# victorramirez952/tomography_3d_reconstructor

Hardware: NVIDIA B200
Metric: Gvoxels/s mask-stack->mesh+volume (higher is better)
Workload: dtype u8 -> bit-packed u32 (topology), f64 field taps -> f32 vertices

## Files before the change

include/t3d.h:

```cpp
#ifndef T3D_H
#define T3D_H

#include <stdint.h>

#ifdef __cplusplus
extern "C" {
#endif

const char* t3d_last_error(void);
int t3d_version(void);
int64_t t3d_words_per_row(int W);
int64_t t3d_launch_count(void);
void t3d_count_launches(int n);


int t3d_pack_masks(const void* masks_u8, int Z, int H, int W, int threshold, void* bits, void* stream);

int t3d_pack_gap(const void* masks_u8, int Z, int H, int W, int threshold, void* bits, void* counts_u64, void* bbox_u32x6,
                 void* stream);

int t3d_unpack_bits(const void* bits, int Z, int H, int W, void* out_u8, void* stream);

int64_t t3d_fill_holes_scratch_bytes(int n_planes, int H, int W);
int t3d_fill_holes_2d(void* bits, int n_planes, int64_t plane_stride_words, int H, int W, void* scratch, void* stream);
// ... 55 lines not shown
int64_t t3d_canonicalize_workspace_bytes(int64_t V, int64_t F);
int t3d_mesh_canonicalize(const void* verts_in, int64_t V, const void* faces_in, int64_t F, void* verts_out,
                          void* faces_out_i64, void* faces_out_i32, void* counts_u64, void* workspace, void* stream);

int64_t t3d_canonicalize_fast_workspace_bytes(int64_t V, int64_t F);
int t3d_mesh_canonicalize_fast_dev(const void* verts_in, int64_t V_cap, const void* V_dev_u64, const void* faces_in, int64_t F_cap,
                                   const void* F_dev_u64, void* verts_out, void* faces_out_i64, void* faces_out_i32,
                                   void* counts_u64, void* workspace, void* stream);
int64_t t3d_canonicalize_structured_workspace_bytes(int64_t V, int64_t F, uint32_t cap_z, uint32_t cap_g0, int Zs);
int t3d_mesh_canonicalize_structured_dev(const void* verts_in, const void* vkeys_u64, int64_t V_cap, const void* sizes_u64,
                                         const void* V_dev_u64, int Zs, int Hs, int Ws, const void* chunkbase_u32,
                                         const void* aw_base_u32, uint32_t aw_stride, int z_offset, int unpad_shift,
                                         const void* cum_f64, const void* adj_f64, int n_cum, int zkey_bits, uint32_t cap_z,
                                         uint32_t cap_g0, const void* faces_in, int64_t F_cap, const void* F_dev_u64,
                                         void* verts_out, void* faces_out_i64, void* faces_out_i32, void* counts_u64,
                                         void* n_g0_u64, void* workspace, int phases, void* stream);

int64_t t3d_mesh_measure_workspace_bytes(void);
int t3d_mesh_measure_dev(const void* verts_f32, const void* faces, int64_t F_cap, const void* F_dev_u64, int faces_are_i64,
                         void* out_f64, void* workspace, void* stream);

int64_t t3d_reconstruct_workspace_bytes(int Z, int H, int W, int add_padding, int n_stages, uint32_t cap_active,
                                        uint32_t cap_verts, uint32_t cap_faces, uint32_t cap_zverts, uint32_t cap_g0);
int64_t t3d_reconstruct_results_len(int Z);
int t3d_reconstruct(const void* masks_u8, int Z, int H, int W, int threshold, int close_ends, int n_stages, unsigned erode_mask,
                    int add_padding, const double* weights3_host, const void* cum_f64, const void* adj_f64, int n_cum,
                    double mm_per_pixel_y, double mm_per_pixel_x, int scale_in_f64, uint32_t cap_active, uint32_t cap_verts,
                    uint32_t cap_faces, uint32_t cap_zverts, uint32_t cap_g0, int zkey_bits, void* verts_out_f32,
                    void* faces_out_i64, void* results_u64, void* workspace, void* stream);

int t3d_slab_pack_gap_ok(const void* masks_u8, int n_own, int H, int W, int threshold);
// ... 70 lines not shown
```

tomography_3d_reconstructor_b200/_lib.py:

```python
from __future__ import annotations

import ctypes
import os

_HERE = os.path.dirname(os.path.abspath(__file__))
LIB_PATH = os.path.join(_HERE, "libt3d.so")

_c = ctypes
_vp, _i, _i64, _u32, _dbl = _c.c_void_p, _c.c_int, _c.c_int64, _c.c_uint32, _c.c_double

class McField(ctypes.Structure):
    _fields_ = [("occ_bits", _vp), ("Z", _i), ("H", _i), ("W", _i), ("pad", _i), ("gaussian", _i), ("weights3_host", _vp),
                ("field_f32", _vp), ("level", _dbl)]


SIGNATURES = {
    "t3d_last_error": (_c.c_char_p, []),
    "t3d_version": (_i, []),
    "t3d_words_per_row": (_i64, [_i]),
    "t3d_launch_count": (_i64, []),
    "t3d_count_launches": (None, [_i]),
    "t3d_pack_masks": (_i, [_vp, _i, _i, _i, _i, _vp, _vp]),
    "t3d_pack_gap": (_i, [_vp, _i, _i, _i, _i, _vp, _vp, _vp, _vp]),
    "t3d_unpack_bits": (_i, [_vp, _i, _i, _i, _vp, _vp]),
# ... 13 lines not shown
    "t3d_field_dense": (_i, [_vp, _i, _i, _i, _i, _i, _vp, _vp, _vp]),
    "t3d_cube_cases": (_i, [_vp, _i, _i, _i, _vp, _vp]),
    "t3d_canonicalize_workspace_bytes": (_i64, [_i64, _i64]),
    "t3d_mesh_canonicalize": (_i, [_vp, _i64, _vp, _i64, _vp, _vp, _vp, _vp, _vp, _vp]),
    "t3d_canonicalize_fast_workspace_bytes": (_i64, [_i64, _i64]),
    "t3d_mesh_measure_workspace_bytes": (_i64, []),
    "t3d_exclusive_scan_u32_dev": (_i, [_vp, _vp, _i64, _i64, _i, _i, _i, _vp, _vp, _vp, _vp]),
    "t3d_mc_words_dev": (_i, [_vp, _i, _i, _i, _i, _i, _vp, _vp, _u32, _vp, _vp, _vp, _vp, _vp, _vp]),
    "t3d_mc_emit_dev": (_i, [_vp, _i, _i, _i, _i, _i, _vp, _vp, _vp, _vp, _u32, _vp, _u32, _u32, _vp, _vp, _i, _vp, _vp]),
    "t3d_mc_vertices_dev": (_i, [_vp, _i, _i, _i, _i, _i, _vp, _vp, _dbl, _vp, _vp, _u32, _i, _i, _vp, _vp, _i, _dbl, _dbl, _i, _i, _vp,
                                 _vp]),
    "t3d_mesh_canonicalize_fast_dev": (_i, [_vp, _i64, _vp, _vp, _i64, _vp, _vp, _vp, _vp, _vp, _vp, _vp]),
    "t3d_mesh_measure_dev": (_i, [_vp, _vp, _i64, _vp, _i, _vp, _vp, _vp]),
    "t3d_canonicalize_structured_workspace_bytes": (_i64, [_i64, _i64, _u32, _u32, _i]),
    "t3d_mesh_canonicalize_structured_dev": (_i, [_vp, _vp, _i64, _vp, _vp, _i, _i, _i, _vp, _vp, _u32, _i, _i, _vp, _vp, _i, _i, _u32,
                                                  _u32, _vp, _i64, _vp, _vp, _vp, _vp, _vp, _vp, _vp, _i, _vp]),
    "t3d_reconstruct_workspace_bytes": (_i64, [_i, _i, _i, _i, _i, _u32, _u32, _u32, _u32, _u32]),
    "t3d_reconstruct_results_len": (_i64, [_i]),
    "t3d_reconstruct": (_i, [_vp, _i, _i, _i, _i, _i, _i, _c.c_uint, _i, _vp, _vp, _vp, _i, _dbl, _dbl, _i, _u32, _u32, _u32,
                             _u32, _u32, _i, _vp, _vp, _vp, _vp, _vp]),
    "t3d_reconstruct_slab_workspace_bytes": (_i64, [_i, _i, _i, _i, _i, _i, _i, _u32, _u32, _u32, _u32, _u32]),
    "t3d_slab_pack_gap_ok": (_i, [_vp, _i, _i, _i, _i]),
    "t3d_slab_pack": (_i, [_vp, _i, _i, _i, _i, _i, _i, _i, _i, _vp, _vp, _vp, _vp, _vp]),
    "t3d_reconstruct_slab": (_i, [_vp, _i, _i, _i, _i, _i, _i, _c.c_uint, _i, _i, _i, _i, _i, _c.c_float, _i, _c.c_float, _i, _vp, _vp,
                                  _vp, _i, _dbl, _dbl, _i, _u32, _u32, _u32, _u32, _u32, _i, _vp, _vp, _vp, _vp, _vp, _vp, _vp]),
    "t3d_slab_stitch_faces": (_i, [_vp, _i64, _vp, _i64, _i, _vp]),
    "t3d_edt_workspace_bytes": (_i64, [_i, _i, _i]),
    "t3d_edt_xy_workspace_bytes": (_i64, [_i, _i, _i]),
    "t3d_edt_xy": (_i, [_vp, _i, _i, _i, _i, _vp, _vp, _vp, _vp]),
    "t3d_edt_z_workspace_bytes": (_i64, [_i, _i, _i]),
    "t3d_edt_z": (_i, [_vp, _vp, _i, _i, _i, _vp, _c.c_float, _i, _vp, _vp, _vp]),
# ... 53 lines not shown
```

tomography_3d_reconstructor_b200/csrc/t3d_common.cuh:

```cuda
#pragma once
#include <cuda_runtime.h>
#include <stdint.h>
#include <stdio.h>

int t3d_num_sms(void);
#define T3D_NUM_SMS (t3d_num_sms())
bool t3d_first_use_on_device(int slot);
enum { T3D_ONCE_FILL_HOLES_ATTR = 0, T3D_ONCE_MC_LUTS = 1, T3D_ONCE_SORT_ATTR = 2, T3D_ONCE_MORPH4_ATTR = 3, T3D_ONCE_SLOTS = 8 };

extern "C" void t3d_set_error(const char* fmt, ...);
extern "C" void t3d_count_launches(int n);
int t3d_zero_async(void* p, size_t n, cudaStream_t st);
void t3d_prezero_register(const void* p, size_t n);
void t3d_prezero_clear(void);
void t3d_canonicalize_structured_zero_range(int64_t V, int64_t F, uint32_t cap_z, uint32_t cap_g0, int Zs, int64_t* offset,
                                            int64_t* size);

#define T3D_CHECK_LAUNCH(name)                                                                   \
    do {                                                                                         \
        cudaError_t e__ = cudaGetLastError();                                                    \
        if (e__ != cudaSuccess) {                                                                \
            t3d_set_error("%s: launch failed: %s", name, cudaGetErrorString(e__));               \
            return 1;                                                                            \
        }                                                                                        \
// ... 120 lines not shown
```

tomography_3d_reconstructor_b200/csrc/t3d_pipeline.cu:

```cuda
#include <stdint.h>

#include <stdlib.h>

#include <nvtx3/nvToolsExt.h>

#include "t3d.h"
#include "t3d_field.cuh"

struct NvtxRange {
    bool open;
    explicit NvtxRange(const char* name) : open(true) { nvtxRangePushA(name); }
    void end() { if (open) { nvtxRangePop(); open = false; } }
    ~NvtxRange() { end(); }
};

enum {
    R_NACTIVE = 0, R_NX = 1, R_NY = 2, R_NZ = 3, R_NT = 4, R_VCANON = 5, R_FCANON = 6, R_UNVERIFIED = 7, R_OVERFLOW = 8,
    R_NAMBIGUOUS = 9, R_NEXACT = 10, R_VOLUME_F64 = 11, R_AREA_F64 = 12, R_BBOX_I32X6 = 13 , R_VRAW = 16, R_NEXC = 17,
    R_NGHOST = 18, R_NLEAD = 19, R_NG0 = 25,
    R_COUNTS = 32
};

#define EXC_CAP (1u << 20)
#define SURF_HALO 3
// ... 335 lines not shown
    r_mc.end();
    marks.mark("vertices", st);
    NvtxRange r_canon("t3d:ensure_manifold_mesh+measures");
    T3D_CUDA(cudaEventRecord(side->e[4], st));
    T3D_CUDA(cudaStreamWaitEvent(side->s, side->e[4], 0));
    RUN(t3d_mc_emit_view_dev(view, x_off, ws + L.sign, Zp, Hp, Wp, g.z_begin, g.z_end, ws + L.ballots, ws + L.chunkbase, ws + L.aw_idx,
                             ws + L.aw_base, cap_active, R + R_NACTIVE, cap_verts, cap_faces, ws + L.vkeys, ws + L.faces_raw, 2, side->s));
    T3D_CUDA(cudaEventRecord(side->e[6], side->s));
    RUN(t3d_mesh_measure_dev(ws + L.verts_raw, ws + L.faces_raw, cap_faces, R + R_NT, 0, R + R_VOLUME_F64, ws + L.measure, side->s));
    T3D_CUDA(cudaEventRecord(side->e[5], side->s));
    t3d_canon_faces_ready_event(side->e[6]);
    if (cap_zverts)
        RUN(t3d_mesh_canonicalize_structured_dev(ws + L.verts_raw, ws + L.vkeys, cap_verts, R + R_NACTIVE, R + R_VRAW, Zp, Hp, Wp,
                                                 ws + L.chunkbase, ws + L.aw_base, cap_active, g.z_offset, 1, cum_f64, adj_f64, n_cum,
                                                 zkey_bits, cap_zverts, cap_g0, ws + L.faces_raw, cap_faces, R + R_NT, verts_out_f32,
                                                 faces_out_i64, nullptr, R + R_VCANON, R + R_NG0, ws + L.canon, 3, st));
    else
        RUN(t3d_mesh_canonicalize_fast_dev(ws + L.verts_raw, cap_verts, R + R_VRAW, ws + L.faces_raw, cap_faces, R + R_NT,
                                           verts_out_f32, faces_out_i64, nullptr, R + R_VCANON, ws + L.canon, st));
    if (t3d_canon_faces_ready_pending()) T3D_CUDA(cudaStreamWaitEvent(st, side->e[6], 0));
    if (g.want_ghost || g.want_lead)
        k_count_plane_vertices<<<1, 64, 0, st>>>((const float*)verts_out_f32, R + R_VCANON, g.z_ghost, g.z_lead, g.want_ghost,
                                                 g.want_lead, R + R_NGHOST, R + R_NLEAD);
    if (g.want_ghost || g.want_lead) t3d_count_launches(1);
    marks.mark("canonicalize", st);
    T3D_CUDA(cudaStreamWaitEvent(st, side->e[5], 0));
    marks.mark("wait measures", st);
    marks.report(st);
    return 0;
}

// ... 275 lines not shown
```

tomography_3d_reconstructor_b200/csrc/t3d_surface.cu:

```cuda
#include <stdlib.h>

#include <cub/device/device_radix_sort.cuh>

#include "t3d_field.cuh"

#define FY 8

__device__ __noinline__ uint32_t exact_sign_bits(const OccView* v, int zp, int yp, int wp, uint32_t need, uint32_t s)
{
    while (need) {
        const int b = __ffs(need) - 1;
        need &= need - 1;
        if (field_value(*v, zp, yp, (wp << 5) + b) > 0.5f) s |= 1u << b; else s &= ~(1u << b);
    }
    return s;
}

__device__ __forceinline__ uint4 prow4(const OccView& v, int zp, int yp, int wp4, uint32_t& left, uint32_t& right)
{
    const int z = zp - v.pad, y = yp - v.pad;
    if (z < 0 || z >= v.Z || y < 0 || y >= v.H) { left = right = 0u; return make_uint4(0, 0, 0, 0); }
    const uint32_t* row = v.bits + (z * v.ps + (long long)y * v.rs);
    const int w0 = 4 * wp4;
    const uint4 o = (w0 < v.nw) ? *reinterpret_cast<const uint4*>(row + w0) : make_uint4(0, 0, 0, 0);
// ... 751 lines not shown

struct CanonS {
    const float* verts;
    const unsigned long long* vkeys;
    const unsigned long long* sizes;
    uint32_t cap_verts, cap_z, cap_g0;
    int Zs, Hs;
    int ncr;
    const uint32_t* chunkbase;
    const uint32_t* aw_base;
    uint32_t stride;
    int g_plane;
    int z_offset; float shift;
    const double* cum; const double* adj; int n_cum;
    int zkey_bits;
    unsigned long long* zkeys;
    uint32_t* zval;
    const uint32_t* zperm;
    unsigned long long* gkeys;
    uint32_t* gval;
    const uint32_t* gperm;
    uint32_t* perm;
    unsigned long long* n_g0_out;
};

template <int AX>
__device__ __forceinline__ uint32_t before_row(const CanonS& c, int64_t row)
{
    const uint32_t na = (uint32_t)c.sizes[0];
    const uint32_t r = row >= (int64_t)c.Zs * c.Hs ? na : c.chunkbase[row * c.ncr];
    return r >= na ? (uint32_t)c.sizes[1 + AX] : c.aw_base[(int64_t)AX * c.stride + r];
}

// ... 30 lines not shown
__device__ __forceinline__ uint32_t canon_zkey(const CanonS& c, uint32_t i, uint32_t nx, uint32_t ny, uint32_t gZ)
{
    if (i < gZ) return 0u;
    const uint32_t raw = nx + ny + i;
    const int k = (int)(c.vkeys[raw] >> 42);
    uint32_t zk = float_key(c.verts[3 * (int64_t)raw]);
    if (c.zkey_bits < 32) {
        const uint32_t base = float_key(plane_z(c, k));
        zk = zk >= base ? zk - base : 0u;
        const uint32_t lim = (1u << c.zkey_bits) - 1u;
        zk = zk > lim ? lim : zk;
    }
    return zk;
}

template <int ZS_U, typename KeyT, typename KeyFn, typename ValFn>
__device__ __forceinline__ void cta_radix_sort_u(uint32_t n, int passes, KeyFn key_of, ValFn value_of, KeyT* keyA, KeyT* keyB, uint32_t* idxA,
                                               uint32_t* idxB, uint32_t* out)
{
    __shared__ uint32_t s_hist[ZS_WARPS][256];
    __shared__ uint32_t s_tot[256];
    __shared__ uint32_t s_carry[8];
    const int tid = threadIdx.x, w = tid >> 5, lane = tid & 31;
    const uint32_t per = (((n + ZS_WARPS - 1) / ZS_WARPS) + 31u) & ~31u;
    const uint32_t ws = min(n, (uint32_t)w * per), we = min(n, ws + per);
    const KeyT* kin = keyA; const uint32_t* iin = idxA;
    KeyT* kout = keyB; uint32_t* iout = idxB;
    for (int p = 0; p < passes; ++p) {
        const int shift = 8 * p;
        const bool first = p == 0, last = p == passes - 1;
        for (int i = tid; i < ZS_WARPS * 256; i += ZS_THREADS) (&s_hist[0][0])[i] = 0;
        __syncthreads();
        for (uint32_t i0 = ws + lane; i0 < we; i0 += 32 * ZS_U) {
            KeyT kk[ZS_U];
#pragma unroll
            for (int u = 0; u < ZS_U; ++u) {
                const uint32_t i = i0 + 32 * u;
                if (i < we) { if (first) { kk[u] = key_of(i); keyA[i] = kk[u]; } else kk[u] = kin[i]; }
            }
#pragma unroll
            for (int u = 0; u < ZS_U; ++u)
                if (i0 + 32 * u < we) atomicAdd(&s_hist[w][(uint32_t)(kk[u] >> shift) & 255u], 1u);
        }
        __syncthreads();
        if (tid < 256) {
            uint32_t t = 0;
            for (int ww = 0; ww < ZS_WARPS; ++ww) t += s_hist[ww][tid];
            s_tot[tid] = t;
        }
        __syncthreads();
        if (tid < 256) {
            const uint32_t v = s_tot[tid];
            const uint32_t incl = warp_incl_scan(v);
            if (lane == 31) s_carry[w] = incl;
            asm volatile("bar.sync 1, 256;" ::: "memory");
            uint32_t carry = 0;
            for (int ww = 0; ww < w; ++ww) carry += s_carry[ww];
            uint32_t run = carry + incl - v;
            for (int ww = 0; ww < ZS_WARPS; ++ww) { const uint32_t h = s_hist[ww][tid]; s_hist[ww][tid] = run; run += h; }
        }
        __syncthreads();
        for (uint32_t c0 = ws; c0 < we; c0 += 32 * ZS_U) {
            KeyT kk[ZS_U];
            uint32_t ii[ZS_U];
#pragma unroll
            for (int u = 0; u < ZS_U; ++u) {
                const uint32_t i = c0 + 32 * u + lane;
                kk[u] = 0; ii[u] = 0;
                if (i < we) {
                    kk[u] = first ? keyA[i] : kin[i];
                    ii[u] = first ? value_of(i) : iin[i];
                }
            }
#pragma unroll
            for (int u = 0; u < ZS_U; ++u) {
                if (c0 + 32 * u >= we) break;
                const uint32_t i = c0 + 32 * u + lane;
                const bool ok = i < we;
                const KeyT key = kk[u];
                const uint32_t idx = ii[u];
                const uint32_t d = ok ? ((uint32_t)(key >> shift) & 255u) : 0xffffffffu;
                const uint32_t peers = __match_any_sync(0xffffffffu, d);
                const uint32_t rank = __popc(peers & ((1u << lane) - 1u));
                uint32_t pos = 0;
                if (ok) pos = s_hist[w][d] + rank;
                __syncwarp();
                if (ok && rank == 0) s_hist[w][d] += __popc(peers);
                __syncwarp();
                if (ok) {
                    if (last) out[pos] = idx;
                    else { kout[pos] = key; iout[pos] = idx; }
                }
            }
        }
        __syncthreads();
        const KeyT* tk = kin; const uint32_t* ti = iin;
        kin = kout; iin = iout;
        kout = (KeyT*)tk; iout = (uint32_t*)ti;
    }
}

template <int ZS_U>
__global__ void __launch_bounds__(ZS_THREADS) k_zsort_layers(CanonS c, uint32_t* __restrict__ keyA, uint32_t* __restrict__ keyB,
                                                            uint32_t* __restrict__ idxA, uint32_t* __restrict__ idxB,
                                                            uint32_t* __restrict__ zperm)
{
    const uint32_t nx = (uint32_t)c.sizes[1], ny = (uint32_t)c.sizes[2], nz = (uint32_t)c.sizes[3];
    if ((unsigned long long)nx + ny + nz > c.cap_verts || nz > c.cap_z) return;
    const int layer = blockIdx.x;
    uint32_t s = before_row<2>(c, (int64_t)layer * c.Hs), e = before_row<2>(c, (int64_t)(layer + 1) * c.Hs);
    if (e > nz) e = nz;
    if (s >= e) return;
    const uint32_t n = e - s;
    uint32_t gX, gY, gZ;
    g0_sizes(c, gX, gY, gZ);
    if (n == 1 || e <= gZ) {
        for (uint32_t i = s + threadIdx.x; i < e; i += ZS_THREADS) zperm[i] = i;
        return;
    }
    cta_radix_sort_u<ZS_U, uint32_t>(n, (c.zkey_bits + 7) / 8, [&](uint32_t i) { return canon_zkey(c, s + i, nx, ny, gZ); },
                                     [&](uint32_t i) { return s + i; }, keyA + s, keyB + s, idxA + s, idxB + s, zperm + s);
}

__global__ void __launch_bounds__(ZS_THREADS) k_gsort(CanonS c, unsigned long long* __restrict__ keyA, unsigned long long* __restrict__ keyB,
                                                     uint32_t* __restrict__ idxA, uint32_t* __restrict__ idxB, uint32_t* __restrict__ gperm)
{
    const uint32_t nx = (uint32_t)c.sizes[1], ny = (uint32_t)c.sizes[2], nz = (uint32_t)c.sizes[3];
    if ((unsigned long long)nx + ny + nz > c.cap_verts) return;
    uint32_t gX, gY, gZ;
    g0_sizes(c, gX, gY, gZ);
    const uint32_t n = gX + gY + gZ;
    if (n == 0 || n > c.cap_g0) return;
    auto raw_of = [&](uint32_t t) -> uint32_t { return t < gX ? t : t < gX + gY ? nx + (t - gX) : nx + ny + (t - gX - gY); };
    if (n == 1) { if (threadIdx.x == 0) gperm[0] = raw_of(0); return; }
    cta_radix_sort_u<1, unsigned long long>(n, 8, [&](uint32_t t) {
        const float* v = c.verts + 3 * (int64_t)raw_of(t);
        return ((unsigned long long)float_key(v[1]) << 32) | float_key(v[2]);
    }, raw_of, keyA, keyB, idxA, idxB, gperm);
}

__global__ void __launch_bounds__(256) k_canon_positions(CanonS c)
{
    __shared__ uint32_t s_g[3];
    const uint32_t i = blockIdx.x * blockDim.x + threadIdx.x;
    const uint32_t nx = (uint32_t)c.sizes[1], ny = (uint32_t)c.sizes[2], nz = (uint32_t)c.sizes[3];
    const unsigned long long V64 = (unsigned long long)nx + ny + nz;
    if (V64 > c.cap_verts) return;
    if (threadIdx.x == 0) g0_sizes(c, s_g[0], s_g[1], s_g[2]);
    __syncthreads();
    if (i >= (uint32_t)V64) return;
    if (nz > c.cap_z) { c.perm[i] = i; return; }
    const uint32_t gX = s_g[0], gY = s_g[1], gZ = s_g[2];
    const uint32_t nG = gX + gY + gZ;
    if (i == 0 && c.n_g0_out) *c.n_g0_out = nG;
    if (i < nG) c.perm[i] = (nG <= c.cap_g0) ? c.gperm[i] : (i < gX ? i : i < gX + gY ? nx + (i - gX) : nx + ny + (i - gX - gY));
    if (i < nx) {
        if (i < gX) return;
        const unsigned long long key = c.vkeys[i];
        const int k = (int)(key >> 42), j = (int)((key >> 22) & 0xfffffu);
        c.perm[i + before_row<1>(c, (int64_t)k * c.Hs + j) + before_row<2>(c, (int64_t)k * c.Hs)] = i;
    } else if (i < nx + ny) {
        const uint32_t iy = i - nx;
        if (iy < gY) return;
        const unsigned long long key = c.vkeys[i];
        const int k = (int)(key >> 42), j = (int)((key >> 22) & 0xfffffu);
        const int64_t row = (int64_t)k * c.Hs + j;
        const uint32_t lo = before_row<1>(c, row), hi = before_row<1>(c, row + 1);
        const uint32_t mine = float_key(c.verts[3 * (int64_t)i + 1]);
        uint32_t r = 0;
        for (uint32_t e = lo; e < hi; ++e) {
            const uint32_t ke = float_key(c.verts[3 * (int64_t)(nx + e) + 1]);
            r += (ke < mine || (ke == mine && e < iy)) ? 1u : 0u;
        }
        c.perm[before_row<0>(c, row + 1) + lo + r + before_row<2>(c, (int64_t)k * c.Hs)] = i;
    } else {
        const uint32_t R = i - nx - ny;
        if (R < gZ) return;
        const uint32_t raw = nx + ny + c.zperm[R];
        const int64_t next_plane = ((int64_t)(c.vkeys[raw] >> 42) + 1) * c.Hs;
        c.perm[before_row<0>(c, next_plane) + before_row<1>(c, next_plane) + R] = raw;
    }
}

extern "C" int64_t t3d_canonicalize_structured_workspace_bytes(int64_t V, int64_t F, uint32_t cap_z, uint32_t cap_g0, int Zs)
{
    const int64_t n = V > F ? V : F;
    int64_t b = 0;
    b += 2 * align256(8 * (int64_t)cap_z) + 2 * align256(4 * (int64_t)cap_z);
    b += 2 * align256(8 * (int64_t)cap_g0) + 2 * align256(4 * (int64_t)cap_g0);
    b += align256(4 * V);
    b += 2 * align256(4 * n);
    b += align256(4 * V);
    b += align256(4 * (int64_t)cap_g0 + 256);
    b += 2 * align256(t3d_scan_workspace_bytes(n, 1)) + 256;
    return b;
}

extern "C" int t3d_canonical_map_offsets(int kind, int64_t V, int64_t F, uint32_t cap_z, uint32_t cap_g0, int Zs, int64_t* out4)
{
    if (V <= 0 || F < 0 || !out4 || kind < 0 || kind > 2) { t3d_set_error("t3d_canonical_map_offsets: bad arguments"); return 2; }
    const int64_t n = V > F ? V : F;
    int64_t o = 0;
    if (kind == 0) {
        out4[1] = 2 * align256(4 * V);
        o = 4 * align256(4 * V);
        out4[2] = o; o += 2 * align256(4 * n);
        out4[0] = o;
        out4[3] = -1;
        return 0;
    }
    if (kind == 1) {
        o = 2 * align256(8 * V) + align256(4 * V);
        out4[1] = o; o += align256(4 * V);
        out4[2] = o; o += 2 * align256(4 * n);
        out4[0] = o; o += align256(4 * V);
        o += align256((int64_t)sort64_temp_bytes(V));
        o += align256(t3d_scan_workspace_bytes(n, 1));
    } else {
        o = 2 * align256(8 * (int64_t)cap_z) + 2 * align256(4 * (int64_t)cap_z) + 2 * align256(8 * (int64_t)cap_g0) +
            2 * align256(4 * (int64_t)cap_g0);
        out4[1] = o; o += align256(4 * V);
        out4[2] = o; o += 2 * align256(4 * n);
        out4[0] = o; o += align256(4 * V);
        o += align256(4 * (int64_t)cap_g0 + 256);
        o += 2 * align256(t3d_scan_workspace_bytes(n, 1));
    }
    out4[3] = o + 8 * 8;
    (void)Zs;
    return 0;
}

void t3d_canonicalize_structured_zero_range(int64_t V, int64_t F, uint32_t cap_z, uint32_t cap_g0, int Zs, int64_t* offset,
                                            int64_t* size)
{
    const int64_t n = V > F ? V : F;
    *size = 2 * align256(t3d_scan_workspace_bytes(n, 1)) + 256;
    *offset = t3d_canonicalize_structured_workspace_bytes(V, F, cap_z, cap_g0, Zs) - *size;
}

extern "C" int t3d_mesh_canonicalize_structured_dev(const void* verts_in, const void* vkeys_u64, int64_t V_cap, const void* sizes_u64,
                                                    const void* V_dev_u64, int Zs, int Hs, int Ws, const void* chunkbase_u32,
                                                    const void* aw_base_u32, uint32_t aw_stride, int z_offset, int unpad_shift,
                                                    const void* cum_f64, const void* adj_f64, int n_cum, int zkey_bits,
                                                    uint32_t cap_z, uint32_t cap_g0, const void* faces_in, int64_t F_cap,
                                                    const void* F_dev_u64, void* verts_out, void* faces_out_i64, void* faces_out_i32,
                                                    void* counts_u64, void* n_g0_u64, void* workspace, int phases, void* stream)
{
    cudaStream_t st = (cudaStream_t)stream;
    if (zkey_bits <= 0 || zkey_bits > 32) zkey_bits = 32;
    if (V_cap <= 0 || V_cap > 0x7fffffff || F_cap < 0 || Zs <= 0 || Hs <= 0 || Ws <= 0 || cap_z == 0 || (phases & 3) == 0) {
        t3d_set_error("t3d_mesh_canonicalize_structured: bad sizes");
        return 2;
    }
    const int64_t V = V_cap, F = F_cap, n = V > F ? V : F;
    char* ws = (char*)workspace;
    CanonS c;
    c.verts = (const float*)verts_in;
    c.vkeys = (const unsigned long long*)vkeys_u64;
    c.sizes = (const unsigned long long*)sizes_u64;
    c.cap_verts = (uint32_t)V; c.cap_z = cap_z; c.cap_g0 = cap_g0;
    c.Zs = Zs; c.Hs = Hs;
    c.ncr = (t3d_wpr(Ws) + 31) >> 5;
    c.chunkbase = (const uint32_t*)chunkbase_u32;
    c.aw_base = (const uint32_t*)aw_base_u32;
    c.stride = aw_stride;
    c.g_plane = (n_cum > 0 && unpad_shift > 0) ? unpad_shift - z_offset : -1;
    c.z_offset = z_offset; c.shift = unpad_shift ? 1.0f : 0.0f;
    c.cum = (const double*)cum_f64; c.adj = (const double*)adj_f64; c.n_cum = n_cum;
    c.zkey_bits = zkey_bits;
    unsigned long long* zkeys_b; uint32_t* zperm; unsigned long long* gkeys_b; uint32_t* gperm;
    c.zkeys = (unsigned long long*)ws; ws += align256(8 * (int64_t)cap_z);
    zkeys_b = (unsigned long long*)ws; ws += align256(8 * (int64_t)cap_z);
    c.zval = (uint32_t*)ws; ws += align256(4 * (int64_t)cap_z);
    zperm = (uint32_t*)ws; ws += align256(4 * (int64_t)cap_z);
    c.gkeys = (unsigned long long*)ws; ws += align256(8 * (int64_t)cap_g0);
    gkeys_b = (unsigned long long*)ws; ws += align256(8 * (int64_t)cap_g0);
    c.gval = (uint32_t*)ws; ws += align256(4 * (int64_t)cap_g0);
    gperm = (uint32_t*)ws; ws += align256(4 * (int64_t)cap_g0);
    c.perm = (uint32_t*)ws; ws += align256(4 * V);
    uint32_t* flags = (uint32_t*)ws; ws += align256(4 * n);
    uint32_t* pos = (uint32_t*)ws; ws += align256(4 * n);
    uint32_t* newid = (uint32_t*)ws; ws += align256(4 * V);
    void* temp = ws; ws += align256(4 * (int64_t)cap_g0 + 256);
    void* scan_ws = ws; ws += align256(t3d_scan_workspace_bytes(n, 1));
    void* scan_ws_f = ws; ws += align256(t3d_scan_workspace_bytes(n, 1));
    unsigned long long* totals = (unsigned long long*)ws;
    unsigned long long* counts = (unsigned long long*)counts_u64;
    c.zperm = zperm; c.gperm = gperm;
    c.n_g0_out = (unsigned long long*)n_g0_u64;
    if (phases & 1) {
        uint32_t* keyA = (uint32_t*)c.zkeys;
        uint32_t* keyB = keyA + cap_z;
        uint32_t* idxA = (uint32_t*)zkeys_b;
        uint32_t* idxB = idxA + cap_z;
        if ((int64_t)cap_z >= 4096 * (int64_t)Zs) k_zsort_layers<8><<<Zs, ZS_THREADS, 0, st>>>(c, keyA, keyB, idxA, idxB, zperm);
        else k_zsort_layers<1><<<Zs, ZS_THREADS, 0, st>>>(c, keyA, keyB, idxA, idxB, zperm);
        t3d_count_launches(1);
    }
    if (phases & 2) {
        if (t3d_zero_async(counts + 2, 8, st)) return 1;
        if (cap_g0 > 0) {
            k_gsort<<<1, ZS_THREADS, 0, st>>>(c, c.gkeys, gkeys_b, c.gval, (uint32_t*)temp, gperm);
        }
        k_canon_positions<<<(unsigned)((V + 255) / 256), 256, 0, st>>>(c);
        if (canonical_tail(c.verts, c.perm, V, (const unsigned long long*)V_dev_u64, faces_in, F, (const unsigned long long*)F_dev_u64,
                           verts_out, faces_out_i64, faces_out_i32, counts, flags, pos, newid, scan_ws, scan_ws_f, totals, st)) return 1;
        t3d_count_launches((F > 0 ? 5 : 3) + (cap_g0 > 0 ? 1 : 0));
    }
    T3D_CHECK_LAUNCH("t3d_mesh_canonicalize_structured");
    return 0;
}

template <typename IdxT>
__global__ void __launch_bounds__(256) k_mesh_measure(const float* __restrict__ verts, const IdxT* __restrict__ faces, int64_t F_cap,
                                                      double* __restrict__ partials, const unsigned long long* __restrict__ F_dev = nullptr)
{
    const int64_t F = dev_n(F_cap, F_dev);
    double vol = 0.0, area = 0.0;
    for (int64_t i = (int64_t)blockIdx.x * blockDim.x + threadIdx.x; i < F; i += (int64_t)gridDim.x * blockDim.x) {
        const float* a = verts + 3 * (int64_t)faces[3 * i];
        const float* b = verts + 3 * (int64_t)faces[3 * i + 1];
        const float* c = verts + 3 * (int64_t)faces[3 * i + 2];
        const double ax = a[0], ay = a[1], az = a[2], bx = b[0], by = b[1], bz = b[2], cx = c[0], cy = c[1], cz = c[2];
// ... 54 lines not shown
```

tomography_3d_reconstructor_b200/engine.py:

```python
from __future__ import annotations

import ctypes
import weakref
from typing import List, Optional, Sequence, Tuple

import numpy as np
import torch

from . import _lib
from ._lib import T3DError, check


class T3DUnavailable(T3DError):
    """libt3d.so or a CUDA device is missing.  Never swallowed by the reference-style `except Exception`."""


def _require_cuda() -> torch.device:
    if not torch.cuda.is_available():
        raise T3DUnavailable("a CUDA device is required: this package has no CPU fallback")
    return torch.device("cuda", torch.cuda.current_device())


def _L():
    try:
# ... 794 lines not shown
def canonicalize_structured(verts, vkeys, faces_i32, sizes, n_z, sign_dims, chunkbase, aw_base, aw_stride, z_offset, unpad_shift,
                            cum_d, adj_d, n_cum, zkey_bits_, sync: bool = True, keep: Optional[dict] = None):
    L = _L()
    V, nT = int(verts.shape[0]), int(faces_i32.shape[0])
    Zs, Hs, Ws = sign_dims
    dev = verts.device
    vout = torch.empty((V, 3), dtype=torch.float32, device=dev)
    fout = torch.empty((nT, 3), dtype=torch.int64, device=dev)
    counts = torch.zeros(4, dtype=torch.int64, device=dev)
    cap_z, cap_g0 = max(n_z, 1), 0
    for _attempt in range(2):
        ws = torch.zeros(int(L.t3d_canonicalize_structured_workspace_bytes(V, nT, cap_z, cap_g0, Zs)) // 8 + 1, dtype=torch.int64, device=dev)
        check(L.t3d_mesh_canonicalize_structured_dev(
            _p(verts), _p(vkeys), V, _p(sizes), None, Zs, Hs, Ws, _p(chunkbase), _p(aw_base), int(aw_stride), int(z_offset),
            int(unpad_shift), _p(cum_d), _p(adj_d), int(n_cum), int(zkey_bits_), cap_z, cap_g0, _p(faces_i32), nT, None,
            _p(vout), _p(fout), None, _p(counts), _p(counts[3:]), _p(ws), 3, _stream()), "t3d_mesh_canonicalize_structured_dev")
        if keep is not None:
            keep["map"] = canonical_map(ws, 2, V, nT, cap_z, cap_g0, Zs)
        if not sync:
            return vout, fout, counts[:3]
        v2, f2, bad, n_g0 = (int(c) for c in counts.cpu().tolist())
        if not bad:
            return vout[:v2], fout[:f2]
        if n_g0 > cap_g0:
            cap_g0 = n_g0 + 16
            continue
        break
    return None


def mesh_measure_async(verts: torch.Tensor, faces: torch.Tensor) -> torch.Tensor:
# ... 55 lines not shown
```

Measured before the change: 851.4.

## Fuse per-layer z-sort and canonical position placement into one kernel

Replaces the separate k_zsort_layers and k_canon_positions kernels with a single per-layer k_canon_layers kernel. It sorts z-vertices per layer, writing their final positions directly through an emit callback, and places x/y vertices using shared-memory row-offset tables. Small layers sort in dynamic shared memory with 16-bit indices instead of global scratch, and large cases split the sort and placement across a second grid dimension. This removes one launch and the zperm round trip through global memory, at the cost of larger shared memory use and per-layer serial work for x/y placement.

```diff
diff --git a/include/t3d.h b/include/t3d.h
--- a/include/t3d.h
+++ b/include/t3d.h
@@ -93,7 +93,7 @@
                                          const void* cum_f64, const void* adj_f64, int n_cum, int zkey_bits, uint32_t cap_z,
                                          uint32_t cap_g0, const void* faces_in, int64_t F_cap, const void* F_dev_u64,
                                          void* verts_out, void* faces_out_i64, void* faces_out_i32, void* counts_u64,
-                                         void* n_g0_u64, void* workspace, int phases, void* stream);
+                                         void* n_g0_u64, void* workspace, void* stream);
 
 int64_t t3d_mesh_measure_workspace_bytes(void);
 int t3d_mesh_measure_dev(const void* verts_f32, const void* faces, int64_t F_cap, const void* F_dev_u64, int faces_are_i64,
diff --git a/tomography_3d_reconstructor_b200/_lib.py b/tomography_3d_reconstructor_b200/_lib.py
--- a/tomography_3d_reconstructor_b200/_lib.py
+++ b/tomography_3d_reconstructor_b200/_lib.py
@@ -51,7 +51,7 @@
     "t3d_mesh_measure_dev": (_i, [_vp, _vp, _i64, _vp, _i, _vp, _vp, _vp]),
     "t3d_canonicalize_structured_workspace_bytes": (_i64, [_i64, _i64, _u32, _u32, _i]),
     "t3d_mesh_canonicalize_structured_dev": (_i, [_vp, _vp, _i64, _vp, _vp, _i, _i, _i, _vp, _vp, _u32, _i, _i, _vp, _vp, _i, _i, _u32,
-                                                  _u32, _vp, _i64, _vp, _vp, _vp, _vp, _vp, _vp, _vp, _i, _vp]),
+                                                  _u32, _vp, _i64, _vp, _vp, _vp, _vp, _vp, _vp, _vp, _vp]),
     "t3d_reconstruct_workspace_bytes": (_i64, [_i, _i, _i, _i, _i, _u32, _u32, _u32, _u32, _u32]),
     "t3d_reconstruct_results_len": (_i64, [_i]),
     "t3d_reconstruct": (_i, [_vp, _i, _i, _i, _i, _i, _i, _c.c_uint, _i, _vp, _vp, _vp, _i, _dbl, _dbl, _i, _u32, _u32, _u32,
diff --git a/tomography_3d_reconstructor_b200/csrc/t3d_common.cuh b/tomography_3d_reconstructor_b200/csrc/t3d_common.cuh
--- a/tomography_3d_reconstructor_b200/csrc/t3d_common.cuh
+++ b/tomography_3d_reconstructor_b200/csrc/t3d_common.cuh
@@ -6,7 +6,7 @@
 int t3d_num_sms(void);
 #define T3D_NUM_SMS (t3d_num_sms())
 bool t3d_first_use_on_device(int slot);
-enum { T3D_ONCE_FILL_HOLES_ATTR = 0, T3D_ONCE_MC_LUTS = 1, T3D_ONCE_SORT_ATTR = 2, T3D_ONCE_MORPH4_ATTR = 3, T3D_ONCE_SLOTS = 8 };
+enum { T3D_ONCE_FILL_HOLES_ATTR = 0, T3D_ONCE_MC_LUTS = 1, T3D_ONCE_CANON_LAYERS_ATTR = 2, T3D_ONCE_MORPH4_ATTR = 3, T3D_ONCE_SLOTS = 8 };
 
 extern "C" void t3d_set_error(const char* fmt, ...);
 extern "C" void t3d_count_launches(int n);
diff --git a/tomography_3d_reconstructor_b200/csrc/t3d_pipeline.cu b/tomography_3d_reconstructor_b200/csrc/t3d_pipeline.cu
--- a/tomography_3d_reconstructor_b200/csrc/t3d_pipeline.cu
+++ b/tomography_3d_reconstructor_b200/csrc/t3d_pipeline.cu
@@ -373,7 +373,7 @@
         RUN(t3d_mesh_canonicalize_structured_dev(ws + L.verts_raw, ws + L.vkeys, cap_verts, R + R_NACTIVE, R + R_VRAW, Zp, Hp, Wp,
                                                  ws + L.chunkbase, ws + L.aw_base, cap_active, g.z_offset, 1, cum_f64, adj_f64, n_cum,
                                                  zkey_bits, cap_zverts, cap_g0, ws + L.faces_raw, cap_faces, R + R_NT, verts_out_f32,
-                                                 faces_out_i64, nullptr, R + R_VCANON, R + R_NG0, ws + L.canon, 3, st));
+                                                 faces_out_i64, nullptr, R + R_VCANON, R + R_NG0, ws + L.canon, st));
     else
         RUN(t3d_mesh_canonicalize_fast_dev(ws + L.verts_raw, cap_verts, R + R_VRAW, ws + L.faces_raw, cap_faces, R + R_NT,
                                            verts_out_f32, faces_out_i64, nullptr, R + R_VCANON, ws + L.canon, st));
diff --git a/tomography_3d_reconstructor_b200/csrc/t3d_surface.cu b/tomography_3d_reconstructor_b200/csrc/t3d_surface.cu
--- a/tomography_3d_reconstructor_b200/csrc/t3d_surface.cu
+++ b/tomography_3d_reconstructor_b200/csrc/t3d_surface.cu
@@ -789,9 +789,6 @@
     int z_offset; float shift;
     const double* cum; const double* adj; int n_cum;
     int zkey_bits;
-    unsigned long long* zkeys;
-    uint32_t* zval;
-    const uint32_t* zperm;
     unsigned long long* gkeys;
     uint32_t* gval;
     const uint32_t* gperm;
@@ -852,22 +849,24 @@
     return zk;
 }
 
-template <int ZS_U, typename KeyT, typename KeyFn, typename ValFn>
-__device__ __forceinline__ void cta_radix_sort_u(uint32_t n, int passes, KeyFn key_of, ValFn value_of, KeyT* keyA, KeyT* keyB, uint32_t* idxA,
-                                               uint32_t* idxB, uint32_t* out)
-{
-    __shared__ uint32_t s_hist[ZS_WARPS][256];
-    __shared__ uint32_t s_tot[256];
-    __shared__ uint32_t s_carry[8];
+struct SortScratch {
+    uint32_t hist[ZS_WARPS][256];
+    uint32_t carry[8];
+};
+
+template <int ZS_U, typename KeyT, typename IdxT, typename KeyFn, typename ValFn, typename EmitFn>
+__device__ __forceinline__ void cta_radix_sort_u(SortScratch& sm, uint32_t n, int passes, KeyFn key_of, ValFn value_of, EmitFn emit,
+                                               KeyT* keyA, KeyT* keyB, IdxT* idxA, IdxT* idxB)
+{
     const int tid = threadIdx.x, w = tid >> 5, lane = tid & 31;
     const uint32_t per = (((n + ZS_WARPS - 1) / ZS_WARPS) + 31u) & ~31u;
     const uint32_t ws = min(n, (uint32_t)w * per), we = min(n, ws + per);
-    const KeyT* kin = keyA; const uint32_t* iin = idxA;
-    KeyT* kout = keyB; uint32_t* iout = idxB;
+    const KeyT* kin = keyA; const IdxT* iin = idxA;
+    KeyT* kout = keyB; IdxT* iout = idxB;
     for (int p = 0; p < passes; ++p) {
         const int shift = 8 * p;
         const bool first = p == 0, last = p == passes - 1;
-        for (int i = tid; i < ZS_WARPS * 256; i += ZS_THREADS) (&s_hist[0][0])[i] = 0;
+        for (int i = tid; i < ZS_WARPS * 256; i += ZS_THREADS) (&sm.hist[0][0])[i] = 0;
         __syncthreads();
         for (uint32_t i0 = ws + lane; i0 < we; i0 += 32 * ZS_U) {
             KeyT kk[ZS_U];
@@ -878,36 +877,31 @@
             }
 #pragma unroll
             for (int u = 0; u < ZS_U; ++u)
-                if (i0 + 32 * u < we) atomicAdd(&s_hist[w][(uint32_t)(kk[u] >> shift) & 255u], 1u);
+                if (i0 + 32 * u < we) atomicAdd(&sm.hist[w][(uint32_t)(kk[u] >> shift) & 255u], 1u);
         }
         __syncthreads();
         if (tid < 256) {
-            uint32_t t = 0;
-            for (int ww = 0; ww < ZS_WARPS; ++ww) t += s_hist[ww][tid];
-            s_tot[tid] = t;
-        }
-        __syncthreads();
-        if (tid < 256) {
-            const uint32_t v = s_tot[tid];
+            uint32_t v = 0;
+            for (int ww = 0; ww < ZS_WARPS; ++ww) v += sm.hist[ww][tid];
             const uint32_t incl = warp_incl_scan(v);
-            if (lane == 31) s_carry[w] = incl;
+            if (lane == 31) sm.carry[w] = incl;
             asm volatile("bar.sync 1, 256;" ::: "memory");
             uint32_t carry = 0;
-            for (int ww = 0; ww < w; ++ww) carry += s_carry[ww];
+            for (int ww = 0; ww < w; ++ww) carry += sm.carry[ww];
             uint32_t run = carry + incl - v;
-            for (int ww = 0; ww < ZS_WARPS; ++ww) { const uint32_t h = s_hist[ww][tid]; s_hist[ww][tid] = run; run += h; }
+            for (int ww = 0; ww < ZS_WARPS; ++ww) { const uint32_t h = sm.hist[ww][tid]; sm.hist[ww][tid] = run; run += h; }
         }
         __syncthreads();
         for (uint32_t c0 = ws; c0 < we; c0 += 32 * ZS_U) {
             KeyT kk[ZS_U];
-            uint32_t ii[ZS_U];
+            IdxT ii[ZS_U];
 #pragma unroll
             for (int u = 0; u < ZS_U; ++u) {
                 const uint32_t i = c0 + 32 * u + lane;
                 kk[u] = 0; ii[u] = 0;
                 if (i < we) {
                     kk[u] = first ? keyA[i] : kin[i];
-                    ii[u] = first ? value_of(i) : iin[i];
+                    ii[u] = first ? (IdxT)value_of(i) : iin[i];
                 }
             }
 #pragma unroll
@@ -916,53 +910,131 @@
                 const uint32_t i = c0 + 32 * u + lane;
                 const bool ok = i < we;
                 const KeyT key = kk[u];
-                const uint32_t idx = ii[u];
+                const IdxT idx = ii[u];
                 const uint32_t d = ok ? ((uint32_t)(key >> shift) & 255u) : 0xffffffffu;
                 const uint32_t peers = __match_any_sync(0xffffffffu, d);
                 const uint32_t rank = __popc(peers & ((1u << lane) - 1u));
                 uint32_t pos = 0;
-                if (ok) pos = s_hist[w][d] + rank;
+                if (ok) pos = sm.hist[w][d] + rank;
                 __syncwarp();
-                if (ok && rank == 0) s_hist[w][d] += __popc(peers);
+                if (ok && rank == 0) sm.hist[w][d] += __popc(peers);
                 __syncwarp();
                 if (ok) {
-                    if (last) out[pos] = idx;
+                    if (last) emit(pos, (uint32_t)idx);
                     else { kout[pos] = key; iout[pos] = idx; }
                 }
             }
         }
         __syncthreads();
-        const KeyT* tk = kin; const uint32_t* ti = iin;
+        const KeyT* tk = kin; const IdxT* ti = iin;
         kin = kout; iin = iout;
-        kout = (KeyT*)tk; iout = (uint32_t*)ti;
-    }
-}
+        kout = (KeyT*)tk; iout = (IdxT*)ti;
+    }
+}
+
+#define CL_SMEM_CAP 8192
+#define CL_SMEM_BYTES (CL_SMEM_CAP * (2 * 4 + 2 * 2))
+#define CL_SMEM_U 4
+static_assert(CL_SMEM_CAP <= 65536, "layer-local indices are 16-bit");
+#define CL_ROW_TAB (CL_SMEM_BYTES / 8)
+#define CL_U 4
 
 template <int ZS_U>
-__global__ void __launch_bounds__(ZS_THREADS) k_zsort_layers(CanonS c, uint32_t* __restrict__ keyA, uint32_t* __restrict__ keyB,
-                                                            uint32_t* __restrict__ idxA, uint32_t* __restrict__ idxB,
-                                                            uint32_t* __restrict__ zperm)
-{
+__global__ void __launch_bounds__(ZS_THREADS, 2) k_canon_layers(CanonS c, uint32_t* __restrict__ keyA, uint32_t* __restrict__ keyB,
+                                                               uint32_t* __restrict__ idxA, uint32_t* __restrict__ idxB)
+{
+    extern __shared__ uint32_t s_dyn[];
+    __shared__ SortScratch s_sort;
+    __shared__ uint32_t s_g[3];
     const uint32_t nx = (uint32_t)c.sizes[1], ny = (uint32_t)c.sizes[2], nz = (uint32_t)c.sizes[3];
-    if ((unsigned long long)nx + ny + nz > c.cap_verts || nz > c.cap_z) return;
-    const int layer = blockIdx.x;
-    uint32_t s = before_row<2>(c, (int64_t)layer * c.Hs), e = before_row<2>(c, (int64_t)(layer + 1) * c.Hs);
-    if (e > nz) e = nz;
-    if (s >= e) return;
-    const uint32_t n = e - s;
-    uint32_t gX, gY, gZ;
-    g0_sizes(c, gX, gY, gZ);
-    if (n == 1 || e <= gZ) {
-        for (uint32_t i = s + threadIdx.x; i < e; i += ZS_THREADS) zperm[i] = i;
+    const unsigned long long V64 = (unsigned long long)nx + ny + nz;
+    if (V64 > c.cap_verts) return;
+    const bool place_xy = gridDim.y == 1 || blockIdx.y == 1, sort_z = gridDim.y == 1 || blockIdx.y == 0;
+    const uint32_t tid = threadIdx.x, gtid = blockIdx.x * ZS_THREADS + tid, gstride = gridDim.x * ZS_THREADS;
+    if (nz > c.cap_z) {
+        if (place_xy)
+            for (uint32_t i = gtid; i < (uint32_t)V64; i += gstride) c.perm[i] = i;
         return;
     }
-    cta_radix_sort_u<ZS_U, uint32_t>(n, (c.zkey_bits + 7) / 8, [&](uint32_t i) { return canon_zkey(c, s + i, nx, ny, gZ); },
-                                     [&](uint32_t i) { return s + i; }, keyA + s, keyB + s, idxA + s, idxB + s, zperm + s);
+    if (tid == 0) g0_sizes(c, s_g[0], s_g[1], s_g[2]);
+    __syncthreads();
+    const uint32_t gX = s_g[0], gY = s_g[1], gZ = s_g[2];
+    const int64_t r0 = (int64_t)blockIdx.x * c.Hs, r1 = r0 + c.Hs;
+    const uint32_t z_below = before_row<2>(c, r0);
+    if (place_xy) {
+        const uint32_t nG = gX + gY + gZ;
+        if (gtid == 0 && c.n_g0_out) *c.n_g0_out = nG;
+        for (uint32_t i = gtid; i < nG; i += gstride)
+            c.perm[i] = (nG <= c.cap_g0) ? c.gperm[i] : (i < gX ? i : i < gX + gY ? nx + (i - gX) : nx + ny + (i - gX - gY));
+        uint32_t* s_b0 = s_dyn;
+        uint32_t* s_b1 = s_dyn + CL_ROW_TAB;
+        const int n_tab = min(c.Hs + 1, CL_ROW_TAB);
+#pragma unroll 4
+        for (int j = tid; j < n_tab; j += ZS_THREADS) { s_b0[j] = before_row<0>(c, r0 + j); s_b1[j] = before_row<1>(c, r0 + j); }
+        __syncthreads();
+        auto b0 = [&](int j) { return j < n_tab ? s_b0[j] : before_row<0>(c, r0 + j); };
+        auto b1 = [&](int j) { return j < n_tab ? s_b1[j] : before_row<1>(c, r0 + j); };
+        auto row_of = [](unsigned long long key) { return (int)((key >> 22) & 0xfffffu); };
+        for (uint32_t i0 = max(b0(0), gX) + tid, e = min(b0(c.Hs), nx); i0 < e; i0 += CL_U * ZS_THREADS) {
+            unsigned long long key[CL_U];
+#pragma unroll
+            for (int u = 0; u < CL_U; ++u) key[u] = i0 + u * ZS_THREADS < e ? c.vkeys[i0 + u * ZS_THREADS] : 0ull;
+#pragma unroll
+            for (int u = 0; u < CL_U; ++u) {
+                const uint32_t i = i0 + u * ZS_THREADS;
+                if (i < e) c.perm[i + b1(row_of(key[u])) + z_below] = i;
+            }
+        }
+        for (uint32_t iy0 = max(b1(0), gY) + tid, e = min(b1(c.Hs), ny); iy0 < e; iy0 += CL_U * ZS_THREADS) {
+            unsigned long long key[CL_U];
+            uint32_t mine[CL_U];
+#pragma unroll
+            for (int u = 0; u < CL_U; ++u) {
+                const uint32_t i = nx + iy0 + u * ZS_THREADS;
+                const bool ok = iy0 + u * ZS_THREADS < e;
+                key[u] = ok ? c.vkeys[i] : 0ull;
+                mine[u] = ok ? float_key(c.verts[3 * (int64_t)i + 1]) : 0u;
+            }
+#pragma unroll
+            for (int u = 0; u < CL_U; ++u) {
+                const uint32_t iy = iy0 + u * ZS_THREADS;
+                if (iy >= e) break;
+                const int j = row_of(key[u]);
+                const uint32_t lo = b1(j), hi = b1(j + 1);
+                uint32_t r = 0;
+                for (uint32_t q = lo; q < hi; ++q) {
+                    const uint32_t kq = float_key(c.verts[3 * (int64_t)(nx + q) + 1]);
+                    r += (kq < mine[u] || (kq == mine[u] && q < iy)) ? 1u : 0u;
+                }
+                c.perm[b0(j + 1) + lo + r + z_below] = nx + iy;
+            }
+        }
+    }
+    if (!sort_z) return;
+    if (place_xy) __syncthreads();
+    const uint32_t s = z_below, e = min(before_row<2>(c, r1), nz);
+    if (s >= e || e <= gZ) return;
+    const uint32_t n = e - s, raw0 = nx + ny + s;
+    uint32_t* out = c.perm + before_row<0>(c, r1) + before_row<1>(c, r1) + s;
+    if (n == 1) { if (tid == 0) out[0] = raw0; return; }
+    const int passes = (c.zkey_bits + 7) / 8;
+    auto key_of = [&](uint32_t i) { return canon_zkey(c, s + i, nx, ny, gZ); };
+    auto value_of = [](uint32_t i) { return i; };
+    auto emit = [&](uint32_t rank, uint32_t i) { out[rank] = raw0 + i; };
+    if (n <= CL_SMEM_CAP) {
+        uint16_t* s_idx = reinterpret_cast<uint16_t*>(s_dyn + 2 * CL_SMEM_CAP);
+        cta_radix_sort_u<CL_SMEM_U, uint32_t, uint16_t>(s_sort, n, passes, key_of, value_of, emit, s_dyn, s_dyn + CL_SMEM_CAP,
+                                                        s_idx, s_idx + CL_SMEM_CAP);
+    } else {
+        cta_radix_sort_u<ZS_U, uint32_t, uint32_t>(s_sort, n, passes, key_of, value_of, emit, keyA + s, keyB + s, idxA + s,
+                                                   idxB + s);
+    }
 }
 
 __global__ void __launch_bounds__(ZS_THREADS) k_gsort(CanonS c, unsigned long long* __restrict__ keyA, unsigned long long* __restrict__ keyB,
                                                      uint32_t* __restrict__ idxA, uint32_t* __restrict__ idxB, uint32_t* __restrict__ gperm)
 {
+    __shared__ SortScratch s_sort;
     const uint32_t nx = (uint32_t)c.sizes[1], ny = (uint32_t)c.sizes[2], nz = (uint32_t)c.sizes[3];
     if ((unsigned long long)nx + ny + nz > c.cap_verts) return;
     uint32_t gX, gY, gZ;
@@ -971,60 +1043,17 @@
     if (n == 0 || n > c.cap_g0) return;
     auto raw_of = [&](uint32_t t) -> uint32_t { return t < gX ? t : t < gX + gY ? nx + (t - gX) : nx + ny + (t - gX - gY); };
     if (n == 1) { if (threadIdx.x == 0) gperm[0] = raw_of(0); return; }
-    cta_radix_sort_u<1, unsigned long long>(n, 8, [&](uint32_t t) {
+    cta_radix_sort_u<1, unsigned long long, uint32_t>(s_sort, n, 8, [&](uint32_t t) {
         const float* v = c.verts + 3 * (int64_t)raw_of(t);
         return ((unsigned long long)float_key(v[1]) << 32) | float_key(v[2]);
-    }, raw_of, keyA, keyB, idxA, idxB, gperm);
-}
-
-__global__ void __launch_bounds__(256) k_canon_positions(CanonS c)
-{
-    __shared__ uint32_t s_g[3];
-    const uint32_t i = blockIdx.x * blockDim.x + threadIdx.x;
-    const uint32_t nx = (uint32_t)c.sizes[1], ny = (uint32_t)c.sizes[2], nz = (uint32_t)c.sizes[3];
-    const unsigned long long V64 = (unsigned long long)nx + ny + nz;
-    if (V64 > c.cap_verts) return;
-    if (threadIdx.x == 0) g0_sizes(c, s_g[0], s_g[1], s_g[2]);
-    __syncthreads();
-    if (i >= (uint32_t)V64) return;
-    if (nz > c.cap_z) { c.perm[i] = i; return; }
-    const uint32_t gX = s_g[0], gY = s_g[1], gZ = s_g[2];
-    const uint32_t nG = gX + gY + gZ;
-    if (i == 0 && c.n_g0_out) *c.n_g0_out = nG;
-    if (i < nG) c.perm[i] = (nG <= c.cap_g0) ? c.gperm[i] : (i < gX ? i : i < gX + gY ? nx + (i - gX) : nx + ny + (i - gX - gY));
-    if (i < nx) {
-        if (i < gX) return;
-        const unsigned long long key = c.vkeys[i];
-        const int k = (int)(key >> 42), j = (int)((key >> 22) & 0xfffffu);
-        c.perm[i + before_row<1>(c, (int64_t)k * c.Hs + j) + before_row<2>(c, (int64_t)k * c.Hs)] = i;
-    } else if (i < nx + ny) {
-        const uint32_t iy = i - nx;
-        if (iy < gY) return;
-        const unsigned long long key = c.vkeys[i];
-        const int k = (int)(key >> 42), j = (int)((key >> 22) & 0xfffffu);
-        const int64_t row = (int64_t)k * c.Hs + j;
-        const uint32_t lo = before_row<1>(c, row), hi = before_row<1>(c, row + 1);
-        const uint32_t mine = float_key(c.verts[3 * (int64_t)i + 1]);
-        uint32_t r = 0;
-        for (uint32_t e = lo; e < hi; ++e) {
-            const uint32_t ke = float_key(c.verts[3 * (int64_t)(nx + e) + 1]);
-            r += (ke < mine || (ke == mine && e < iy)) ? 1u : 0u;
-        }
-        c.perm[before_row<0>(c, row + 1) + lo + r + before_row<2>(c, (int64_t)k * c.Hs)] = i;
-    } else {
-        const uint32_t R = i - nx - ny;
-        if (R < gZ) return;
-        const uint32_t raw = nx + ny + c.zperm[R];
-        const int64_t next_plane = ((int64_t)(c.vkeys[raw] >> 42) + 1) * c.Hs;
-        c.perm[before_row<0>(c, next_plane) + before_row<1>(c, next_plane) + R] = raw;
-    }
+    }, raw_of, [&](uint32_t rank, uint32_t raw) { gperm[rank] = raw; }, keyA, keyB, idxA, idxB);
 }
 
 extern "C" int64_t t3d_canonicalize_structured_workspace_bytes(int64_t V, int64_t F, uint32_t cap_z, uint32_t cap_g0, int Zs)
 {
     const int64_t n = V > F ? V : F;
     int64_t b = 0;
-    b += 2 * align256(8 * (int64_t)cap_z) + 2 * align256(4 * (int64_t)cap_z);
+    b += 2 * align256(8 * (int64_t)cap_z);
     b += 2 * align256(8 * (int64_t)cap_g0) + 2 * align256(4 * (int64_t)cap_g0);
     b += align256(4 * V);
     b += 2 * align256(4 * n);
@@ -1055,8 +1084,7 @@
         o += align256((int64_t)sort64_temp_bytes(V));
         o += align256(t3d_scan_workspace_bytes(n, 1));
     } else {
-        o = 2 * align256(8 * (int64_t)cap_z) + 2 * align256(4 * (int64_t)cap_z) + 2 * align256(8 * (int64_t)cap_g0) +
-            2 * align256(4 * (int64_t)cap_g0);
+        o = 2 * align256(8 * (int64_t)cap_z) + 2 * align256(8 * (int64_t)cap_g0) + 2 * align256(4 * (int64_t)cap_g0);
         out4[1] = o; o += align256(4 * V);
         out4[2] = o; o += 2 * align256(4 * n);
         out4[0] = o; o += align256(4 * V);
@@ -1082,11 +1110,11 @@
                                                     const void* cum_f64, const void* adj_f64, int n_cum, int zkey_bits,
                                                     uint32_t cap_z, uint32_t cap_g0, const void* faces_in, int64_t F_cap,
                                                     const void* F_dev_u64, void* verts_out, void* faces_out_i64, void* faces_out_i32,
-                                                    void* counts_u64, void* n_g0_u64, void* workspace, int phases, void* stream)
+                                                    void* counts_u64, void* n_g0_u64, void* workspace, void* stream)
 {
     cudaStream_t st = (cudaStream_t)stream;
     if (zkey_bits <= 0 || zkey_bits > 32) zkey_bits = 32;
-    if (V_cap <= 0 || V_cap > 0x7fffffff || F_cap < 0 || Zs <= 0 || Hs <= 0 || Ws <= 0 || cap_z == 0 || (phases & 3) == 0) {
+    if (V_cap <= 0 || V_cap > 0x7fffffff || F_cap < 0 || Zs <= 0 || Hs <= 0 || Ws <= 0 || cap_z == 0) {
         t3d_set_error("t3d_mesh_canonicalize_structured: bad sizes");
         return 2;
     }
@@ -1106,11 +1134,9 @@
     c.z_offset = z_offset; c.shift = unpad_shift ? 1.0f : 0.0f;
     c.cum = (const double*)cum_f64; c.adj = (const double*)adj_f64; c.n_cum = n_cum;
     c.zkey_bits = zkey_bits;
-    unsigned long long* zkeys_b; uint32_t* zperm; unsigned long long* gkeys_b; uint32_t* gperm;
-    c.zkeys = (unsigned long long*)ws; ws += align256(8 * (int64_t)cap_z);
-    zkeys_b = (unsigned long long*)ws; ws += align256(8 * (int64_t)cap_z);
-    c.zval = (uint32_t*)ws; ws += align256(4 * (int64_t)cap_z);
-    zperm = (uint32_t*)ws; ws += align256(4 * (int64_t)cap_z);
+    uint32_t* zkeys = (uint32_t*)ws; ws += align256(8 * (int64_t)cap_z);
+    uint32_t* zidx = (uint32_t*)ws; ws += align256(8 * (int64_t)cap_z);
+    unsigned long long* gkeys_b; uint32_t* gperm;
     c.gkeys = (unsigned long long*)ws; ws += align256(8 * (int64_t)cap_g0);
     gkeys_b = (unsigned long long*)ws; ws += align256(8 * (int64_t)cap_g0);
     c.gval = (uint32_t*)ws; ws += align256(4 * (int64_t)cap_g0);
@@ -1124,27 +1150,23 @@
     void* scan_ws_f = ws; ws += align256(t3d_scan_workspace_bytes(n, 1));
     unsigned long long* totals = (unsigned long long*)ws;
     unsigned long long* counts = (unsigned long long*)counts_u64;
-    c.zperm = zperm; c.gperm = gperm;
+    c.gperm = gperm;
     c.n_g0_out = (unsigned long long*)n_g0_u64;
-    if (phases & 1) {
-        uint32_t* keyA = (uint32_t*)c.zkeys;
-        uint32_t* keyB = keyA + cap_z;
-        uint32_t* idxA = (uint32_t*)zkeys_b;
-        uint32_t* idxB = idxA + cap_z;
-        if ((int64_t)cap_z >= 4096 * (int64_t)Zs) k_zsort_layers<8><<<Zs, ZS_THREADS, 0, st>>>(c, keyA, keyB, idxA, idxB, zperm);
-        else k_zsort_layers<1><<<Zs, ZS_THREADS, 0, st>>>(c, keyA, keyB, idxA, idxB, zperm);
-        t3d_count_launches(1);
-    }
-    if (phases & 2) {
-        if (t3d_zero_async(counts + 2, 8, st)) return 1;
-        if (cap_g0 > 0) {
-            k_gsort<<<1, ZS_THREADS, 0, st>>>(c, c.gkeys, gkeys_b, c.gval, (uint32_t*)temp, gperm);
-        }
-        k_canon_positions<<<(unsigned)((V + 255) / 256), 256, 0, st>>>(c);
-        if (canonical_tail(c.verts, c.perm, V, (const unsigned long long*)V_dev_u64, faces_in, F, (const unsigned long long*)F_dev_u64,
-                           verts_out, faces_out_i64, faces_out_i32, counts, flags, pos, newid, scan_ws, scan_ws_f, totals, st)) return 1;
-        t3d_count_launches((F > 0 ? 5 : 3) + (cap_g0 > 0 ? 1 : 0));
-    }
+    if (t3d_zero_async(counts + 2, 8, st)) return 1;
+    if (cap_g0 > 0) {
+        k_gsort<<<1, ZS_THREADS, 0, st>>>(c, c.gkeys, gkeys_b, c.gval, (uint32_t*)temp, gperm);
+    }
+    if (t3d_first_use_on_device(T3D_ONCE_CANON_LAYERS_ATTR)) {
+        T3D_CUDA(cudaFuncSetAttribute(k_canon_layers<1>, cudaFuncAttributeMaxDynamicSharedMemorySize, CL_SMEM_BYTES));
+        T3D_CUDA(cudaFuncSetAttribute(k_canon_layers<8>, cudaFuncAttributeMaxDynamicSharedMemorySize, CL_SMEM_BYTES));
+    }
+    if ((int64_t)cap_z >= 4096 * (int64_t)Zs)
+        k_canon_layers<8><<<dim3(Zs, 2), ZS_THREADS, CL_SMEM_BYTES, st>>>(c, zkeys, zkeys + cap_z, zidx, zidx + cap_z);
+    else
+        k_canon_layers<1><<<Zs, ZS_THREADS, CL_SMEM_BYTES, st>>>(c, zkeys, zkeys + cap_z, zidx, zidx + cap_z);
+    if (canonical_tail(c.verts, c.perm, V, (const unsigned long long*)V_dev_u64, faces_in, F, (const unsigned long long*)F_dev_u64,
+                       verts_out, faces_out_i64, faces_out_i32, counts, flags, pos, newid, scan_ws, scan_ws_f, totals, st)) return 1;
+    t3d_count_launches((F > 0 ? 5 : 2) + (cap_g0 > 0 ? 1 : 0));
     T3D_CHECK_LAUNCH("t3d_mesh_canonicalize_structured");
     return 0;
 }
diff --git a/tomography_3d_reconstructor_b200/engine.py b/tomography_3d_reconstructor_b200/engine.py
--- a/tomography_3d_reconstructor_b200/engine.py
+++ b/tomography_3d_reconstructor_b200/engine.py
@@ -832,7 +832,7 @@
         check(L.t3d_mesh_canonicalize_structured_dev(
             _p(verts), _p(vkeys), V, _p(sizes), None, Zs, Hs, Ws, _p(chunkbase), _p(aw_base), int(aw_stride), int(z_offset),
             int(unpad_shift), _p(cum_d), _p(adj_d), int(n_cum), int(zkey_bits_), cap_z, cap_g0, _p(faces_i32), nT, None,
-            _p(vout), _p(fout), None, _p(counts), _p(counts[3:]), _p(ws), 3, _stream()), "t3d_mesh_canonicalize_structured_dev")
+            _p(vout), _p(fout), None, _p(counts), _p(counts[3:]), _p(ws), _stream()), "t3d_mesh_canonicalize_structured_dev")
         if keep is not None:
             keep["map"] = canonical_map(ws, 2, V, nT, cap_z, cap_g0, Zs)
         if not sync:
```

Result: faster. 868.3, median of 6 (+2.0%).
